# Gustavroot/DeflatedMLMC_Schwinger

Measured on AMD Instinct MI355X. Metric: hutchinson_probe_samples_per_sec_schwinger128, higher is better.
Workload: dtype f64

## Files before the change

### deflatedmlmc_schwinger_amd/csrc/sw_engine.hip

```cpp
#include "../../include/schwinger_hip.h"
#include "sw_kernels.hpp"
#include "sw_pack.hpp"
#include "sw_poly.hpp"

#include <dlfcn.h>

#include <algorithm>
#include <chrono>
#include <cmath>
#include <complex>
#include <cstdarg>
#include <cstdio>
#include <cstdlib>
#include <cstring>
#include <functional>
#include <map>
#include <mutex>
#include <string>
#include <type_traits>
#include <vector>

using swk::cplx;
using swk::cplxf;
using swk::PtrList;
// ... 157 lines not shown
  bool direct_small = true;
  bool lgmres_aug = true;
  bool stencil_nt = false;
  int stencil_tile = 0;
  int stencil_spw = 0;
  bool cgs2 = false;
  bool verify = true;
  bool inner_cgs2 = false;
  bool pyth_last = true;
  bool eo_solve = true;
  bool eo_direct = true;
  bool precond_f32 = false;
  int kd = 0;
  cplx* U = nullptr;
  int defl_gemm = 0;
  int lkd[SW_MAX_LEVELS] = {0};
  cplx* lV[SW_MAX_LEVELS] = {nullptr};
  int* perm_src[SW_MAX_LEVELS] = {nullptr};
  EllOp rhsmap[SW_MAX_LEVELS];
  cplx* partial = nullptr;
  size_t partial_bytes = 0;
  cplx* small = nullptr;
  size_t small_bytes = 0;
  void* stage = nullptr;
  size_t stage_bytes = 0;
  std::vector<std::pair<void*, size_t>> allocs;
  int pb_level = -1, pb_nb = 0, pb_nbp = 0;
  int8_t* pb_probes = nullptr;
  struct ProbeSlot {
    int8_t* p = nullptr;
    size_t bytes = 0;
    int level = -1, nb = 0;
    hipEvent_t ready = nullptr;
    bool pending = false;
  };
  std::vector<ProbeSlot> slots;
  bool mt_set = false;
  uint32_t* mt_win0 = nullptr;
  uint32_t* mt_win = nullptr;
  int mt_cur = 0;
  uint64_t mt_pos = 0;
  uint32_t* mt_poly = nullptr;
  uint64_t mt_dist = 0;
  uint32_t* mt_family = nullptr;
  uint64_t mt_fam_seg = 0;
  int mt_fam_count = 0;
// ... 6 lines not shown
  bool profiling = false;
  std::vector<EventRec> recs;
  std::vector<hipEvent_t> evpool;
  double tacc[T_NCAT] = {0};
  int64_t tcount[T_NCAT] = {0};
  double twork[T_NCAT] = {0};
  int64_t launches = 0;
  int* d_notconv = nullptr;
  int nc_next = 0;
  int* h_notconv = nullptr;
  int* d_tick = nullptr;
  bool fused_reduce = true;
  double stop_factor = 1.0;
  std::vector<double> direct_relres;
  int64_t direct_fallbacks = 0;
  double alloc_s = 0.0, alloc_bytes = 0.0;
  int64_t alloc_calls = 0, pool_hits = 0;
  cplx* eig_buf[3] = {nullptr, nullptr, nullptr};
  signed char* eig_sign = nullptr;
  cplx* eig_small = nullptr;
  int eig_w = 64;
  cplx* eig_cs[2] = {nullptr, nullptr};
  int eig_hid = -1, eig_level = -1, eig_n = 0;
  void* comm = nullptr;
  double* d_stats = nullptr;
};

static int g_dot_blocks = 1024, g_dot_pmax = 1024;

struct EngineOption {
// ... 29 lines not shown
    field<&sw_engine::dense_map>("dense_map", [](double v) { return (int)v >= 0 && (int)v <= 3; },
                                 "dense_map must be 0..3"),
    field<&sw_engine::bsr_sub>("bsr_sub", [](double v) { return (int)v >= 1; }, "bsr_sub must be >= 1"),
    field<&sw_engine::bsr_stages>("bsr_stages", [](double v) { return v == 2.0 || v == 4.0 || v == 8.0; },
                                  "bsr_stages must be 2, 4 or 8 (dense_stages: or 16)"),
    field<&sw_engine::dense_stages>("dense_stages",
                                    [](double v) { return v == 2.0 || v == 4.0 || v == 8.0 || v == 16.0; },
                                    "dense_stages must be 2, 4 or 8 (dense_stages: or 16)"),
    field<&sw_engine::bsr_nt>("bsr_nt"),
    field<&sw_engine::bsr_xreg>("bsr_xreg"),
    {"dense_lds", get_field<&sw_engine::dense_lds>,
     [](sw_engine* h, double v) { h->dense_lds = v == 1.0 ? 2 : (int)v; },
     [](double v) { return v == 0.0 || v == 1.0 || v == 2.0 || v == 4.0; }, "dense_lds must be 0, 2 or 4"},
    field<&sw_engine::defl_gemm>("defl_gemm", [](double v) { return v == 0.0 || v == 1.0; },
                                 "defl_gemm must be 0 or 1"),
    field<&sw_engine::fused_reduce>("fused_reduce"),
    {"dot_blocks", [](const sw_engine*) { return (double)g_dot_blocks; },
     [](sw_engine*, double v) { g_dot_blocks = g_dot_pmax = std::max(64, (int)v); }},
    field<&sw_engine::gj_block>("gj_block",
                                [](double v) {
                                  const int b = (int)v;
                                  return b == 0 || (b >= 8 && b <= 256 && b % 8 == 0);
                                },
                                "gj_block must be 0 or a multiple of 8 in 8..256"),
    field<&sw_engine::stencil_nt>("stencil_nt"),
    field<&sw_engine::stencil_tile>("stencil_tile"),
    field<&sw_engine::stencil_spw>("stencil_spw",
                                   [](double v) {
                                     const int t = (int)v;
                                     return t == 0 || t == 1 || t == 2 || t == 4 || t == 8;
// ... 25 lines not shown
                                   "stop_factor must be in (0, 1]"),
    field<&sw_engine::precond_f32>("precond_f32"),
    field<&sw_engine::f32_krylov>("f32_krylov"),
    field<&sw_engine::f32_pairs>("f32_pairs"),
    field<&sw_engine::f32_tiles>("f32_tiles",
                                 [](double v) { const int t = (int)v; return t == 0 || t == 1 || t == 2 || t == 4; },
                                 "f32_tiles must be 0, 1, 2 or 4"),
    field<&sw_engine::f32_stages>("f32_stages"),
    field<&sw_engine::f32_dense_stages>("f32_dense_stages"),
    field<&sw_engine::f32_splitk>("f32_splitk"),
    field<&sw_engine::bench_what>("bench_what", [](double v) { return !(v < 0.0 || v > 3.0); },
                                  "bench_what must be 0..3"),
    field<&sw_engine::bench_mode>("bench_mode", [](double v) { return v == 0.0 || v == 1.0 || v == 2.0; },
                                  "bench_mode must be 0, 1 or 2"),
    {"direct_fallbacks", get_field<&sw_engine::direct_fallbacks>, nullptr},
    {"alloc_seconds", get_field<&sw_engine::alloc_s>, nullptr},
    {"alloc_calls", get_field<&sw_engine::alloc_calls>, nullptr},
    {"alloc_gbytes", [](const sw_engine* h) { return h->alloc_bytes * 1e-9; }, nullptr},
    {"pool_hits", get_field<&sw_engine::pool_hits>, nullptr},
};

static int sw_fail(sw_engine* h, const char* fmt, ...) {
  char buf[1024];
  va_list ap;
  va_start(ap, fmt);
  vsnprintf(buf, sizeof buf, fmt, ap);
  va_end(ap);
  if (h) h->err = buf;
  else g_create_error = buf;
  return 1;
// ... 864 lines not shown
      const bool even = lv.stencil ? (row < lv.n / 2) : (even_row_tile[row / 16] != 0);
      if (even) ev.push_back(g);
    }
    if (ev.empty()) continue;
    SWCHK(upload(h, &P.order_even, ev.data(), ev.size()));
    P.ngroups_even = (int)ev.size();
  }
  H.even_valid = true;
  return 0;
}

static inline int* sink_slot(sw_engine* h);
static bool f32_capable(const Hier& H, int level);

static int gram_cycle(sw_engine* h, const KrylovSys& sys, const cplx* R, cplx* X, int L, KrylovWS& ws, int nbp,
                      swk::FgTail tg) {
  const size_t vec = (size_t)sys.n * nbp;
  PtrList pu, pz;
  pu.p[0] = R;
  for (int j = 0; j < L; ++j) {
    cplx* z = ws.Z + vec * j;
    cplx* w = ws.V + vec * j;
    SWCHK(sys.precond(pu.p[j], z));
    SWCHK(sys.apply(0, z, nullptr, w));
    pu.p[j + 1] = w;
    pz.p[j] = z;
  }
  tg.kind = SW_TAIL_GRAM;
  tg.s = ws.sc;
  tg.j = L;
  tg.h1 = ws.gram;
  SWCHK(multigram(h, pu, L + 1, sys.n, nbp, ws.gram, &tg));
  return multiaxpy(h, pz, L, ws.sc.ys, 1.0, X, X, sys.n, nbp, nullptr);
}

static int kcycle_gram(sw_engine* h, Hier& H, int level, const cplx* B, cplx* X, int L, KrylovWS& ws, int nbp) {
  swk::FgTail tg{};
  tg.first_cycle = 1;
  tg.notconv = sink_slot(h);
  SWCHK(zero_vec(h, X, H.lv[level].n, nbp));
  return gram_cycle(h, full_system(h, H, level, nbp, true, false), B, X, L, ws, nbp, tg);
}

static int coarse_correction(sw_engine* h, Hier& H, int l, int nbp) {
  Level& lv = H.lv[l];
  Level& lc = H.lv[l + 1];
  const int last = H.nlevels - 1;
  if (lv.kcycle > 0 && l + 1 < last) {
// ... 520 lines not shown
  const int hid_idx = (int)(&H - &h->hier[0]);
  const int check_from = (outer && h->lazy_sync) ? std::max(0, h->sync_hint[hid_idx][level] - 2) : 0;
  const int n = sys.n;
  const size_t vec = (size_t)n * nbp;
  const int tb = 256, tg = (nbp + tb - 1) / tb;
  const double tol_stop = outer ? tol * h->stop_factor : tol;
  const bool z32 = (bool)sys.precond32;
  const bool k32 = z32 && h->f32_krylov;
  if (aug && (outer || sys.precond || ws.m < m + 1)) return sw_fail(h, "internal: augmented cycle misused");
  if (z32 && !(k32 ? (bool)sys.op32 : (bool)sys.op32w))
    return sw_fail(h, "internal: complex64 operator of the Krylov system missing");
  int done = 0;
  bool first = true;
  bool converged = false;
  if (outer) SWCHK(reset_slots(h));
  SWCHK(zero_vec(h, X, n, nbp));
  const cplx* Rcur = B;
  if (z32) {
    Level& lv = H.lv[level];
    SWCHK(ensure_f32(h, H));
    SWCHK(ensure_level_ws32(h, lv, nbp));
    const size_t full = (size_t)lv.n * nbp;
    if (!ws.Z32) {
      SWCHK(dev_realloc(h, &ws.Z32, full * m));
      SWCHK(dev_realloc(h, &ws.v32, full));
    }
    if (k32 && !ws.V32) SWCHK(dev_realloc(h, &ws.V32, full * m));
  }
  while (done < maxiter && !converged) {
    {
      PtrList pl;
// ... 58 lines not shown
      }
      }
      if (outer && tol_stop > 0.0 && (done + j + 1 >= check_from || done + j + 1 >= maxiter ||
                                      ((done + j + 1) & 7) == 0)) {
        int left = 0;
        SWCHK(read_slot(h, slot, &left));
        if (left == 0) {
          converged = true;
          ++j;
          break;
        }
      }
    }
    const int k = j;
    SWCHK(launch(h, T_OTHER, swk::k_fg_solve, dim3(tg), dim3(tb), ws.sc, k));
    if (z32) {
      swk::PtrListT<cplxf> pz;
      for (int q = 0; q < k; ++q) pz.p[q] = ws.Z32 + vec * q;
      SWCHK(multiaxpy(h, pz, k, ws.sc.ys, 1.0, X, X, n, nbp, nullptr));
    } else {
      PtrList pz;
      for (int q = 0; q < k; ++q) pz.p[q] = ws.Z + vec * q;
      SWCHK(multiaxpy(h, pz, k, ws.sc.ys, 1.0, X, X, n, nbp, nullptr));
    }
    done += k;
    first = false;
    if (!outer) break;
    if (converged && h->verify) {
      SWCHK(sys.apply(1, X, B, ws.rres));
      PtrList pr;
      pr.p[0] = ws.rres;
      int* slot = nullptr;
      SWCHK(take_slot(h, &slot));
      const swk::FgTail tv = tail_verify(ws, tol, tol_stop, slot);
      SWCHK(multidot(h, pr, 1, ws.rres, n, nbp, ws.nrm, nullptr, nullptr, &tv));
      int left = 0;
      SWCHK(read_slot(h, slot, &left));
      if (left != 0) {
// ... 202 lines not shown
  if (hid == 0) {
    h->kd = 0;
    SWCHK(dev_free(h, h->U));
    h->U = nullptr;
    for (int l = 0; l < SW_MAX_LEVELS; ++l) {
      h->lkd[l] = 0;
      SWCHK(dev_free(h, h->lV[l]));
      h->lV[l] = nullptr;
      SWCHK(dev_free(h, h->perm_src[l]));
      h->perm_src[l] = nullptr;
      SWCHK(free_op(h, h->rhsmap[l]));
    }
    HIPCHK(hipStreamSynchronize(h->gen_stream));
    for (auto& sl : h->slots) {
      SWCHK(dev_free(h, sl.p));
      if (sl.ready) (void)hipEventDestroy(sl.ready);
    }
    h->slots.clear();
    h->pb_slot = -1;
    h->pb_probes = nullptr;
    h->pb_level = -1;
    h->pb_nb = h->pb_nbp = 0;
    h->pb_ws_nbp = 0;
  }
  return 0;
}

int sw_set_lattice(sw_engine* h, int hid, int L, double mass, const double* U1, const double* U2) {
  SWCHK(check_hier(h, hid, 0, false));
  if (L < 2 || (L & 1)) return sw_fail(h, "lattice extent L=%d must be even and >= 2", L);
// ... 1371 lines not shown
  if (h->precond_f32 && h->f32_krylov && f32_capable(H, 0)) {
    s.precond32 = [h, &H, nbp](const cplxf* v, cplxf* z) { return vcycle32_even(h, H, v, z, nbp); };
    s.op32 = [h, &lv, nbp](const cplxf* z, cplxf* w) { return schur_apply32(h, lv, z, w, nbp); };
  }
  return s;
}

static int reduced_rhs(sw_engine* h, Level& lv, const cplx* B, KrylovWS& ws, int nbp) {
  PtrList pl;
  pl.p[0] = B;
  const swk::FgTail tbeg = tail_begin(ws, 1);
  SWCHK(multidot(h, pl, 1, B, lv.n, nbp, ws.nrm, nullptr, nullptr, &tbeg));
  return eo_hop<0>(h, lv, B, B, ws.xacc, nbp);
}

static int fgmres_eo(sw_engine* h, Hier& H, const cplx* B, cplx* X, double tol, int maxiter, int m,
                     KrylovWS& ws, int nbp, int* iters_total) {
  Level& lv = H.lv[0];
  SWCHK(ensure_level_ws(h, lv, nbp));
  SWCHK(reduced_rhs(h, lv, B, ws, nbp));
  SWCHK(fgmres_loop(h, H, 0, reduced_system(h, H, nbp), ws.xacc, X, tol, maxiter, m, true, ws, nbp,
                    iters_total));
  return eo_hop<1>(h, lv, B, X, X, nbp);
}

static int fgmres_eo_gram(sw_engine* h, Hier& H, const cplx* B, cplx* X, double tol, int maxiter, int m,
                          KrylovWS& ws, int nbp, int* iters_total) {
  Level& lv = H.lv[0];
  const int hid_idx = (int)(&H - &h->hier[0]);
  const int hint = h->lazy_sync ? h->sync_hint[hid_idx][0] : 0;
  const KrylovSys sys = reduced_system(h, H, nbp);
  const double tol_stop = tol * h->stop_factor;
  SWCHK(ensure_level_ws(h, lv, nbp));
  SWCHK(reset_slots(h));
  SWCHK(reduced_rhs(h, lv, B, ws, nbp));
  const cplx* bp = ws.xacc;
  SWCHK(zero_vec(h, X, sys.n, nbp));
  std::vector<std::complex<double>> hrr(nbp), hrr0(nbp);
  int done = 0;
  bool converged = false;
  const cplx* Rcur = bp;
  int L = std::min(m, maxiter);
  while (done < maxiter && !converged) {
    L = std::max(1, std::min(L, std::min(m, maxiter - done)));
    int* slot = nullptr;
    SWCHK(take_slot(h, &slot));
    swk::FgTail tg{};
    tg.tol = tol;
    tg.tol_stop = tol_stop;
    tg.iter_base = done;
    tg.notconv = slot;
    SWCHK(gram_cycle(h, sys, Rcur, X, L, ws, nbp, tg));
    done += L;
    SWCHK(sys.apply(1, X, bp, ws.rres));
    Rcur = ws.rres;
    const bool observe = tol_stop > 0.0 && (hint <= 0 || done + m >= hint || done >= maxiter);
    int Lnext = m;
    if (observe) {
      int left = 0;
      SWCHK(read_slot(h, slot, &left));
      if (left == 0) {
        converged = true;
      } else {
        HIPCHK(hipMemcpy(hrr.data(), ws.sc.relres, sizeof(cplx) * nbp, hipMemcpyDeviceToHost));
        HIPCHK(hipMemcpy(hrr0.data(), ws.sc.g, sizeof(cplx) * nbp, hipMemcpyDeviceToHost));
        double need = 1.0;
        for (int c = 0; c < nbp; ++c) {
// ... 9 lines not shown
      PtrList pr;
      pr.p[0] = ws.rres;
      int* vslot = nullptr;
      SWCHK(take_slot(h, &vslot));
      const swk::FgTail tv = tail_verify(ws, tol, tol_stop, vslot);
      SWCHK(multidot(h, pr, 1, ws.rres, sys.n, nbp, ws.nrm, nullptr, nullptr, &tv));
      int left = 0;
      SWCHK(read_slot(h, vslot, &left));
      if (left != 0) {
        converged = false;
        Lnext = 1;
      }
    }
    L = Lnext;
  }
  SWCHK(eo_hop<1>(h, lv, B, X, X, nbp));
  if (iters_total) *iters_total = done;
  h->sync_hint[hid_idx][0] = converged ? done : 0;
  return 0;
}

static bool level_is_direct(sw_engine* h, Hier& H, int level) {
  return h->direct_small && level < H.nlevels - 1 && !H.lv[level].stencil && H.lv[level].dinv.set &&
         h->use_mfma;
}

static int solve_dev(sw_engine* h, int hid, int level0, const cplx* B, cplx* X, double tol,
                     int maxiter, int nbp, int* total) {
  Hier& H = h->hier[hid];
  Level& lv = H.lv[level0];
  if (level0 == H.nlevels - 1 && H.nlevels > 1) {
    SWCHK(apply_coarsest(h, H, B, X, nbp));
    if (total) *total = 1;
    return 0;
// ... 22 lines not shown
        worst = std::max(worst, rr);
      }
      if (!(worst > tol * h->stop_factor)) return 0;
      if (pass == 3) break;
      SWCHK(launch_bsr(h, lv.dinv, 0, lv.r, nullptr, lv.t, nbp, T_COARSEST, cplx{0.0, 0.0}));
      SWCHK(vec_add(h, X, lv.t, X, lv.n, nbp));
    }
    h->direct_relres.clear();
    h->direct_fallbacks++;
    const int mfb = std::min(h->restart, std::max(1, maxiter));
    SWCHK(ensure_krylov(h, lv.sws, mfb, lv.n, nbp, true));
    return fgmres(h, H, level0, B, X, tol, maxiter, mfb, true, lv.sws, nbp, total);
  }
  const int m = std::min(h->restart, std::max(1, maxiter));
  SWCHK(ensure_krylov(h, lv.sws, m, lv.n, nbp, true));
  if (eo_solve_eligible(h, H, level0)) {
    const bool k32 = h->precond_f32 && h->f32_krylov && f32_capable(H, 0);
    int P = 0, rpb = 0;
    row_blocking(lv.n / 2, nbp, true, &P, &rpb);
    if (h->gram_cycle && !k32 && m <= SW_GRAM_MAXL && fused_ok(h, P, nbp))
      return fgmres_eo_gram(h, H, B, X, tol, maxiter, m, lv.sws, nbp, total);
    return fgmres_eo(h, H, B, X, tol, maxiter, m, lv.sws, nbp, total);
  }
  return fgmres(h, H, level0, B, X, tol, maxiter, m, true, lv.sws, nbp, total);
}

static int fetch_iters(sw_engine* h, KrylovWS& ws, int nb, int32_t* iters, double* relres,
                       int fallback_iters) {
  std::vector<int> it(ws.nbp);
  std::vector<std::complex<double>> rr(ws.nbp);
  HIPCHK(hipMemcpy(it.data(), ws.sc.iters, sizeof(int) * ws.nbp, hipMemcpyDeviceToHost));
  HIPCHK(hipMemcpy(rr.data(), ws.sc.relres, sizeof(cplx) * ws.nbp, hipMemcpyDeviceToHost));
  for (int j = 0; j < nb; ++j) {
    if (iters) iters[j] = it[j] >= 0 ? it[j] : fallback_iters;
    if (relres) relres[j] = rr[j].real();
  }
  return 0;
}
// ... 38 lines not shown
  SWCHK(dev_realloc(h, &h->pb_x0, cnt));
  SWCHK(dev_realloc(h, &h->pb_rhs, cnt));
  SWCHK(dev_realloc(h, &h->pb_z, cnt));
  SWCHK(dev_realloc(h, &h->pb_xc, cnt));
  SWCHK(dev_realloc(h, &h->pb_xc2, cnt));
  SWCHK(dev_realloc(h, &h->pb_y, cnt));
  SWCHK(dev_realloc(h, &h->pb_w, cnt));
  SWCHK(dev_realloc(h, &h->pb_w2, cnt));
  SWCHK(dev_realloc(h, &h->pb_xd, cnt));
  SWCHK(dev_realloc(h, &h->pb_est, (size_t)4 * nbp));
  SWCHK(dev_realloc(h, &h->pb_iters, (size_t)2 * nbp));
  h->pb_ws_nbp = nbp;
  return 0;
}

int sw_probes_upload_slot(sw_engine* h, int slot, int level, int nb, const int8_t* probes) {
  SWCHK(check_hier(h, 0, level, true));
  if (nb <= 0 || !probes) return sw_fail(h, "bad arguments");
  if (slot < 0 || slot >= 4096) return sw_fail(h, "probe slot %d out of range", slot);
  HIPCHK(hipSetDevice(h->device));
  Level& lv = h->hier[0].lv[level];
  const size_t bytes = (size_t)nb * lv.n;
  if ((int)h->slots.size() <= slot) h->slots.resize(slot + 1);
  sw_engine::ProbeSlot& sl = h->slots[slot];
  if (sl.pending) {
    HIPCHK(hipStreamSynchronize(h->gen_stream));
    sl.pending = false;
  }
  if (sl.bytes < bytes) {
    SWCHK(dev_free(h, sl.p));
    sl.p = nullptr;
    void* q;
    SWCHK(dev_alloc(h, &q, bytes));
    sl.p = (int8_t*)q;
    sl.bytes = bytes;
  }
  HIPCHK(hipMemcpyAsync(sl.p, probes, bytes, hipMemcpyHostToDevice, h->stream));
  HIPCHK(hipStreamSynchronize(h->stream));
  sl.level = level;
  sl.nb = nb;
  return 0;
}

int sw_probes_select(sw_engine* h, int slot) {
  if (!h) return 1;
  if (slot < 0 || slot >= (int)h->slots.size() || !h->slots[slot].p)
    return sw_fail(h, "probe slot %d is empty", slot);
  h->pb_slot = slot;
  h->pb_probes = h->slots[slot].p;
  h->pb_level = h->slots[slot].level;
  h->pb_nb = h->slots[slot].nb;
  h->pb_nbp = pad64(h->pb_nb);
  return 0;
}

// ... 86 lines not shown
    void* q;
    SWCHK(dev_alloc(h, &q, total));
    sl.p = (int8_t*)q;
    sl.bytes = total;
  }
  {
    LaunchScope ls(h, T_OTHER);
    hipLaunchKernelGGL(swk::k_mt_generate, dim3(S), dim3(SW_MT_BLOCK), 0, gs,
                       (const uint32_t*)(h->mt_win + (size_t)SW_MT_N * h->mt_cur),
                       (const uint32_t*)h->mt_family, (unsigned long long)segdraws,
                       (unsigned long long)total, kind, sl.p);
    KLAUNCH_CHECK();
  }
  sl.level = level;
  sl.nb = nb;
  if (!sl.ready) HIPCHK(hipEventCreateWithFlags(&sl.ready, hipEventDisableTiming));
  HIPCHK(hipEventRecord(sl.ready, gs));
  sl.pending = true;
  return 0;
}

int sw_probes_fetch(sw_engine* h, int slot, int8_t* out) {
  if (!h) return 1;
  if (!out) return sw_fail(h, "null output");
  if (slot < 0 || slot >= (int)h->slots.size() || !h->slots[slot].p)
    return sw_fail(h, "probe slot %d is empty", slot);
  HIPCHK(hipSetDevice(h->device));
  SWCHK(stream_sync(h));
  HIPCHK(hipStreamSynchronize(h->gen_stream));
  const sw_engine::ProbeSlot& sl = h->slots[slot];
// ... 3 lines not shown
}

static int dot_into(sw_engine* h, const cplx* A, const cplx* Bv, int n, int nbp, cplx* out) {
  PtrList pl;
  pl.p[0] = A;
  return multidot(h, pl, 1, Bv, n, nbp, out);
}

static int record_iters(sw_engine* h, KrylovWS* ws, int total_or_const, std::vector<int32_t>& dst,
                        int nb) {
  dst.assign(nb, total_or_const);
  if (ws) {
    std::vector<int> it(ws->nbp);
    HIPCHK(hipMemcpy(it.data(), ws->sc.iters, sizeof(int) * ws->nbp, hipMemcpyDeviceToHost));
    for (int j = 0; j < nb; ++j) dst[j] = it[j] >= 0 ? it[j] : total_or_const;
  }
  return 0;
}

static int deflate(sw_engine* h, const cplx* U, int kd, const int* srcrow, const cplx* X, cplx* out,
                   int n, int nbp) {
  const int ld = defl_ld(kd);
  cplx* cbuf = h->small + 8 * nbp;
  if (h->defl_gemm || kd > 64) {
    const int nchunks = nbp / 16;
    const int pmax = std::max(1, (n + 63) / 64);
    int P = std::max(1, std::min(pmax, 2048 / nchunks));
    const int rpb = (n + P - 1) / P;
    P = (n + rpb - 1) / rpb;
    SWCHK(ensure_partial(h, (size_t)P * ld * nbp * sizeof(cplx)));
    SWCHK(pick_ge<64, 128, 256>(ld, [&](auto LD) {
      return launch(h, T_DEFL, swk::k_defl_gemm_dots<LD / 64>, dim3(P, nchunks), dim3(SW_BLOCK), U, ld, X, n, nbp,
                    rpb, h->partial);
    }));
    SWCHK(launch(h, T_DEFL, swk::k_reduce_partials, dim3(ld, nbp / 64), dim3(SW_BLOCK), h->partial, P, ld, nbp,
                 cbuf, (const cplx*)nullptr, (cplx*)nullptr));
    return launch(h, T_DEFL, swk::k_defl_gemm_apply, dim3((n + 63) / 64, nbp / 64), dim3(SW_BLOCK), U, ld,
                  (const cplx*)cbuf, srcrow, X, out, n, nbp);
  }
  int P, rpb;
  row_blocking(n, nbp, true, &P, &rpb);
  for (int k0 = 0; k0 < kd; k0 += 32) {
    const int kc = std::min(32, kd - k0);
    SWCHK(ensure_partial(h, (size_t)P * kc * nbp * sizeof(cplx)));
    SWCHK(pick_ge<8, 16, 32>(kc, [&](auto KC) {
      return launch(h, T_DEFL, swk::k_defl_dots<KC>, dim3(P, nbp / 64), dim3(SW_BLOCK), (const cplx*)(U + k0), ld,
                    kc, X, n, nbp, rpb, h->partial);
    }));
    SWCHK(launch(h, T_DEFL, swk::k_reduce_partials, dim3(kc, nbp / 64), dim3(SW_BLOCK), h->partial, P, kc, nbp,
                 cbuf + (size_t)k0 * nbp, (const cplx*)nullptr, (cplx*)nullptr));
  }
  {
    dim3 grid((n + SW_WAVES_PER_BLOCK - 1) / SW_WAVES_PER_BLOCK, nbp / 64);
    SWCHK(launch(h, T_DEFL, swk::k_defl_apply, grid, dim3(SW_BLOCK), U, ld, kd, cbuf, srcrow, X, out, n, nbp));
  }
  return 0;
}

int sw_apply_deflation(sw_engine* h, int which, int level, int nb, const double* X, double* Y) {
  SWCHK(check_hier(h, 0, level, false));
  if (which != 0 && which != 1) return sw_fail(h, "which must be 0 (Hutchinson) or 1 (MLMC level)");
  if (which == 0 && level != 0) return sw_fail(h, "the Hutchinson deflation acts at level 0");
  if (nb <= 0 || !X || !Y) return sw_fail(h, "bad arguments");
  const int kd = which == 0 ? h->kd : h->lkd[level];
  const cplx* U = which == 0 ? h->U : h->lV[level];
  if (kd <= 0 || !U) return sw_fail(h, "no deflation vectors registered at level %d", level);
  HIPCHK(hipSetDevice(h->device));
  Level& lv = h->hier[0].lv[level];
  const int nbp = pad64(nb);
  cplx *a, *b;
  SWCHK(io_vectors(h, lv, nbp, &a, &b));
  SWCHK(ensure_small(h, nbp));
  SWCHK(pack_host(h, lv, nb, X, a, nbp));
  SWCHK(deflate(h, U, kd, which == 0 ? (const int*)h->perm_src[0] : nullptr, a, b, lv.n, nbp));
  return unpack_host(h, lv, nb, b, Y, nbp);
}

int sw_hutch_run(sw_engine* h, int mode, int level, double tol, int maxiter) {
  SWCHK(check_hier(h, 0, level, true));
  if (h->pb_level != level || h->pb_nb <= 0) return sw_fail(h, "no probes uploaded for level %d", level);
  if (maxiter < 1) return sw_fail(h, "maxiter must be >= 1");
  HIPCHK(hipSetDevice(h->device));
  Hier& H0 = h->hier[0];
  const int nb = h->pb_nb, nbp = h->pb_nbp;
  Level& lv = H0.lv[level];
  const int n = lv.n;
  SWCHK(ensure_probe_ws(h, nbp));
  SWCHK(ensure_small(h, nbp));
  if (h->pb_slot >= 0 && h->pb_slot < (int)h->slots.size() && h->slots[h->pb_slot].pending) {
    HIPCHK(hipStreamWaitEvent(h->stream, h->slots[h->pb_slot].ready, 0));
    h->slots[h->pb_slot].pending = false;
  }
  SWCHK(launch(h, T_OTHER, swk::k_pack_i8, dim3((n + 63) / 64, nbp / 64), dim3(SW_BLOCK), h->pb_probes, nb, n,
               (const int*)lv.rowmap, h->pb_x0, nbp));
  const int fine_hid = (level == 0 && h->hier[h->solver_hid].ready) ? h->solver_hid : 0;
  if (fine_hid != 0 && h->hier[fine_hid].lv[0].n != n)
    return sw_fail(h, "solver hierarchy level-0 size mismatch");
  if (mode == SW_MODE_HUTCHINSON) {
    if (level != 0) return sw_fail(h, "Hutchinson mode runs at level 0");
    const int kd = h->kd;
    if (kd > 0) {
      SWCHK(deflate(h, h->U, kd, (const int*)h->perm_src[0], h->pb_x0, h->pb_rhs, n, nbp));
    } else {
      dim3 grid((n + SW_WAVES_PER_BLOCK - 1) / SW_WAVES_PER_BLOCK, nbp / 64);
      SWCHK(launch(h, T_DEFL, swk::k_gather_rows, grid, dim3(SW_BLOCK), (const int*)h->perm_src[0], h->pb_x0,
                   h->pb_rhs, n, nbp));
    }
    int total = 0;
    SWCHK(solve_dev(h, fine_hid, 0, h->pb_rhs, h->pb_z, tol, maxiter, nbp, &total));
    SWCHK(dot_into(h, h->pb_x0, h->pb_z, n, nbp, h->pb_est));
    SWCHK(stream_sync(h));
    SWCHK(record_iters(h, &h->hier[fine_hid].lv[0].sws, total, h->last_iters_f, nb));
// ... 283 lines not shown
```

### deflatedmlmc_schwinger_amd/csrc/sw_kernels.hpp

```cpp
#pragma once
#include <hip/hip_runtime.h>
#include <stdint.h>

namespace swk {

typedef double2 cplx;

#define SW_WAVE 64
#define SW_BLOCK 256
#define SW_WAVES_PER_BLOCK 4

__device__ __forceinline__ cplx cmake(double a, double b) { cplx r; r.x = a; r.y = b; return r; }
__device__ __forceinline__ cplx cadd(cplx a, cplx b) { return cmake(a.x + b.x, a.y + b.y); }
__device__ __forceinline__ cplx csub(cplx a, cplx b) { return cmake(a.x - b.x, a.y - b.y); }
__device__ __forceinline__ cplx cmul(cplx a, cplx b) {
  return cmake(fma(a.x, b.x, -a.y * b.y), fma(a.x, b.y, a.y * b.x));
}
__device__ __forceinline__ cplx cmulc(cplx a, cplx b) {
  return cmake(fma(a.x, b.x, a.y * b.y), fma(a.x, b.y, -a.y * b.x));
}
__device__ __forceinline__ void cfma(cplx& acc, cplx a, cplx b) {
  acc.x = fma(a.x, b.x, acc.x);
  acc.x = fma(-a.y, b.y, acc.x);
  acc.y = fma(a.x, b.y, acc.y);
// ... 2131 lines not shown
  const int r1 = min(n, r0 + rows_per_block);
  cplx c[KT];
#pragma unroll
  for (int k = 0; k < KT; ++k) {
    c[k] = cmake(0.0, 0.0);
    if (k < K) {
      const cplx t = coef[(size_t)k * nbp + col];
      c[k] = cmake(sign * t.x, sign * t.y);
    }
  }
  double nrm = 0.0;
  constexpr int UNR = (sizeof(CV) == sizeof(cplxf) && sizeof(CW) == sizeof(cplxf)) ? 4 : 2;
#pragma unroll UNR
  for (int r = r0 + wave; r < r1; r += SW_WAVES_PER_BLOCK) {
    const size_t off = (size_t)r * nbp + col;
    cplx w = widen(Win[off]);
#pragma unroll
    for (int k = 0; k < KT; ++k)
      if (k < K) cfma(w, c[k], widen(V.p[k][off]));
    Wout[off] = narrow<CW>(w);
    if (W32) W32[off] = cmake((float)w.x, (float)w.y);
    if (NORM) nrm = fma(w.x, w.x, fma(w.y, w.y, nrm));
  }
  if (NORM) {
    if (wave > 0) redn[wave - 1][lane] = nrm;
    __syncthreads();
    if (wave == 0) {
      nrm += redn[0][lane];
      nrm += redn[1][lane];
      nrm += redn[2][lane];
      st_partial(&partial[(size_t)blockIdx.x * nbp + col], cmake(nrm, 0.0), ra.tick1 != nullptr);
// ... 36 lines not shown
  const size_t stride = (size_t)gridDim.x * blockDim.x;
  for (; i < count; i += stride) dst[i] = cadd(a[i], b[i]);
}

__global__ __launch_bounds__(SW_BLOCK) void k_gather_rows(const int* __restrict__ srcrow,
                                                          const cplx* __restrict__ src,
                                                          cplx* __restrict__ dst, int n, int nbp) {
  const int wave = threadIdx.x >> 6, lane = threadIdx.x & 63;
  const size_t col = (size_t)blockIdx.y * 64 + lane;
  const int r = blockIdx.x * SW_WAVES_PER_BLOCK + wave;
  if (r >= n) return;
  const int s = srcrow ? srcrow[r] : r;
  dst[(size_t)r * nbp + col] = src[(size_t)s * nbp + col];
}

template <int KT>
__global__ __launch_bounds__(SW_BLOCK) void k_defl_dots(const cplx* __restrict__ U, int ldu,
                                                        int kd, const cplx* __restrict__ X, int n,
                                                        int nbp, int rows_per_block,
                                                        cplx* __restrict__ partial) {
  __shared__ cplx red[3][8][64];
  const int wave = threadIdx.x >> 6, lane = threadIdx.x & 63;
  const size_t col = (size_t)blockIdx.y * 64 + lane;
  const int r0 = blockIdx.x * rows_per_block;
  const int r1 = min(n, r0 + rows_per_block);
  cplx acc[KT];
#pragma unroll
  for (int k = 0; k < KT; ++k) acc[k] = cmake(0.0, 0.0);
  for (int r = r0 + wave; r < r1; r += SW_WAVES_PER_BLOCK) {
    const int ru = __builtin_amdgcn_readfirstlane(r);
    const cplx x = X[(size_t)ru * nbp + col];
    const cplx* u = U + (size_t)ru * ldu;
#pragma unroll
    for (int k = 0; k < KT; ++k)
      if (k < kd) cfmac(acc[k], u[k], x);
  }
  for (int kb = 0; kb < KT; kb += 8) {
    if (kb >= kd) break;
    if (wave > 0) {
#pragma unroll
      for (int k = 0; k < 8; ++k)
        if (kb + k < KT) red[wave - 1][k][lane] = acc[kb + k];
    }
    __syncthreads();
    if (wave == 0) {
#pragma unroll
// ... 17 lines not shown
                                                         const cplx* __restrict__ X,
                                                         cplx* __restrict__ out, int n, int nbp) {
  const int wave = threadIdx.x >> 6, lane = threadIdx.x & 63;
  const size_t col = (size_t)blockIdx.y * 64 + lane;
  const int r = __builtin_amdgcn_readfirstlane(blockIdx.x * SW_WAVES_PER_BLOCK + wave);
  if (r >= n) return;
  const int s = srcrow ? srcrow[r] : r;
  cplx x = X[(size_t)s * nbp + col];
  const cplx* u = U + (size_t)s * ldu;
#pragma unroll 4
  for (int k = 0; k < kd; ++k) {
    const cplx ck = c[(size_t)k * nbp + col];
    cfma(x, cmake(-u[k].x, -u[k].y), ck);
  }
  out[(size_t)r * nbp + col] = x;
}

template <int KT>
__global__ __launch_bounds__(SW_BLOCK) void k_defl_gemm_dots(const cplx* __restrict__ U, int ldu,
                                                             const cplx* __restrict__ X, int n, int nbp,
                                                             int rows_per_block,
                                                             cplx* __restrict__ partial) {
  const int lane = threadIdx.x & 63, wave = threadIdx.x >> 6;
  const int k = lane >> 4, c = lane & 15;
  const int t0 = wave * KT;
  const int nt = min(KT, ldu / 16 - t0);
  if (nt <= 0) return;
  const int r0 = blockIdx.x * rows_per_block;
  const int r1 = min(n, r0 + rows_per_block);
  const size_t j = (size_t)blockIdx.y * 16 + c;
// ... 436 lines not shown
```

Measured before the change: 35450.

## Add fused Hutchinson probe path with int8 probe image and fused deflation/EO kernels

Adds a dedicated Hutchinson path for level 0. Probe vectors stay in a pre-transposed, row-mapped int8 image built when probes are uploaded, possibly on the generator stream. Deflation dots read the int8 probes directly. A fused kernel builds the deflated, even-odd reduced right-hand side together with its norm, and another fused kernel reconstructs the odd sites and accumulates the trace estimate. This replaces the separate pack, deflate-apply, reduced-rhs, hop and dot launches and their full complex-vector traffic. The first FGMRES cycle also skips zeroing X and reading it back in the axpy. The cost is more kernel code, an extra per-slot buffer, and an eligibility check that falls back to the old path.

```diff
diff --git a/deflatedmlmc_schwinger_amd/csrc/sw_engine.hip b/deflatedmlmc_schwinger_amd/csrc/sw_engine.hip
--- a/deflatedmlmc_schwinger_amd/csrc/sw_engine.hip
+++ b/deflatedmlmc_schwinger_amd/csrc/sw_engine.hip
@@ -195,6 +195,7 @@
   int kd = 0;
   cplx* U = nullptr;
   int defl_gemm = 0;
+  bool probe_path = true;
   int lkd[SW_MAX_LEVELS] = {0};
   cplx* lV[SW_MAX_LEVELS] = {nullptr};
   int* perm_src[SW_MAX_LEVELS] = {nullptr};
@@ -211,6 +212,9 @@
   struct ProbeSlot {
     int8_t* p = nullptr;
     size_t bytes = 0;
+    int8_t* xt = nullptr;
+    size_t xt_bytes = 0;
+    bool xt_ok = false;
     int level = -1, nb = 0;
     hipEvent_t ready = nullptr;
     bool pending = false;
@@ -247,6 +251,7 @@
   double stop_factor = 1.0;
   std::vector<double> direct_relres;
   int64_t direct_fallbacks = 0;
+  int64_t probe_batches = 0;
   double alloc_s = 0.0, alloc_bytes = 0.0;
   int64_t alloc_calls = 0, pool_hits = 0;
   cplx* eig_buf[3] = {nullptr, nullptr, nullptr};
@@ -306,6 +311,7 @@
      [](double v) { return v == 0.0 || v == 1.0 || v == 2.0 || v == 4.0; }, "dense_lds must be 0, 2 or 4"},
     field<&sw_engine::defl_gemm>("defl_gemm", [](double v) { return v == 0.0 || v == 1.0; },
                                  "defl_gemm must be 0 or 1"),
+    field<&sw_engine::probe_path>("probe_path"),
     field<&sw_engine::fused_reduce>("fused_reduce"),
     {"dot_blocks", [](const sw_engine*) { return (double)g_dot_blocks; },
      [](sw_engine*, double v) { g_dot_blocks = g_dot_pmax = std::max(64, (int)v); }},
@@ -361,6 +367,7 @@
     field<&sw_engine::bench_mode>("bench_mode", [](double v) { return v == 0.0 || v == 1.0 || v == 2.0; },
                                   "bench_mode must be 0, 1 or 2"),
     {"direct_fallbacks", get_field<&sw_engine::direct_fallbacks>, nullptr},
+    {"probe_batches", get_field<&sw_engine::probe_batches>, nullptr},
     {"alloc_seconds", get_field<&sw_engine::alloc_s>, nullptr},
     {"alloc_calls", get_field<&sw_engine::alloc_calls>, nullptr},
     {"alloc_gbytes", [](const sw_engine* h) { return h->alloc_bytes * 1e-9; }, nullptr},
@@ -1255,7 +1262,7 @@
 static bool f32_capable(const Hier& H, int level);
 
 static int gram_cycle(sw_engine* h, const KrylovSys& sys, const cplx* R, cplx* X, int L, KrylovWS& ws, int nbp,
-                      swk::FgTail tg) {
+                      swk::FgTail tg, bool first = false) {
   const size_t vec = (size_t)sys.n * nbp;
   PtrList pu, pz;
   pu.p[0] = R;
@@ -1272,7 +1279,7 @@
   tg.j = L;
   tg.h1 = ws.gram;
   SWCHK(multigram(h, pu, L + 1, sys.n, nbp, ws.gram, &tg));
-  return multiaxpy(h, pz, L, ws.sc.ys, 1.0, X, X, sys.n, nbp, nullptr);
+  return multiaxpy(h, pz, L, ws.sc.ys, 1.0, first ? (const cplx*)nullptr : X, X, sys.n, nbp, nullptr);
 }
 
 static int kcycle_gram(sw_engine* h, Hier& H, int level, const cplx* B, cplx* X, int L, KrylovWS& ws, int nbp) {
@@ -1823,7 +1830,7 @@
   bool first = true;
   bool converged = false;
   if (outer) SWCHK(reset_slots(h));
-  SWCHK(zero_vec(h, X, n, nbp));
+  if (!outer) SWCHK(zero_vec(h, X, n, nbp));
   const cplx* Rcur = B;
   if (z32) {
     Level& lv = H.lv[level];
@@ -1912,14 +1919,15 @@
     }
     const int k = j;
     SWCHK(launch(h, T_OTHER, swk::k_fg_solve, dim3(tg), dim3(tb), ws.sc, k));
+    const cplx* x0 = (outer && first) ? nullptr : X;
     if (z32) {
       swk::PtrListT<cplxf> pz;
       for (int q = 0; q < k; ++q) pz.p[q] = ws.Z32 + vec * q;
-      SWCHK(multiaxpy(h, pz, k, ws.sc.ys, 1.0, X, X, n, nbp, nullptr));
+      SWCHK(multiaxpy(h, pz, k, ws.sc.ys, 1.0, x0, X, n, nbp, nullptr));
     } else {
       PtrList pz;
       for (int q = 0; q < k; ++q) pz.p[q] = ws.Z + vec * q;
-      SWCHK(multiaxpy(h, pz, k, ws.sc.ys, 1.0, X, X, n, nbp, nullptr));
+      SWCHK(multiaxpy(h, pz, k, ws.sc.ys, 1.0, x0, X, n, nbp, nullptr));
     }
     done += k;
     first = false;
@@ -2152,6 +2160,7 @@
     HIPCHK(hipStreamSynchronize(h->gen_stream));
     for (auto& sl : h->slots) {
       SWCHK(dev_free(h, sl.p));
+      SWCHK(dev_free(h, sl.xt));
       if (sl.ready) (void)hipEventDestroy(sl.ready);
     }
     h->slots.clear();
@@ -3553,28 +3562,20 @@
   return eo_hop<0>(h, lv, B, B, ws.xacc, nbp);
 }
 
-static int fgmres_eo(sw_engine* h, Hier& H, const cplx* B, cplx* X, double tol, int maxiter, int m,
-                     KrylovWS& ws, int nbp, int* iters_total) {
-  Level& lv = H.lv[0];
-  SWCHK(ensure_level_ws(h, lv, nbp));
-  SWCHK(reduced_rhs(h, lv, B, ws, nbp));
-  SWCHK(fgmres_loop(h, H, 0, reduced_system(h, H, nbp), ws.xacc, X, tol, maxiter, m, true, ws, nbp,
-                    iters_total));
-  return eo_hop<1>(h, lv, B, X, X, nbp);
-}
-
-static int fgmres_eo_gram(sw_engine* h, Hier& H, const cplx* B, cplx* X, double tol, int maxiter, int m,
-                          KrylovWS& ws, int nbp, int* iters_total) {
-  Level& lv = H.lv[0];
+static int fgmres_eo_loop(sw_engine* h, Hier& H, cplx* X, double tol, int maxiter, int m, KrylovWS& ws, int nbp,
+                          int* iters_total) {
+  return fgmres_loop(h, H, 0, reduced_system(h, H, nbp), ws.xacc, X, tol, maxiter, m, true, ws, nbp,
+                     iters_total);
+}
+
+static int fgmres_eo_gram_loop(sw_engine* h, Hier& H, cplx* X, double tol, int maxiter, int m, KrylovWS& ws,
+                               int nbp, int* iters_total) {
   const int hid_idx = (int)(&H - &h->hier[0]);
   const int hint = h->lazy_sync ? h->sync_hint[hid_idx][0] : 0;
   const KrylovSys sys = reduced_system(h, H, nbp);
   const double tol_stop = tol * h->stop_factor;
-  SWCHK(ensure_level_ws(h, lv, nbp));
   SWCHK(reset_slots(h));
-  SWCHK(reduced_rhs(h, lv, B, ws, nbp));
   const cplx* bp = ws.xacc;
-  SWCHK(zero_vec(h, X, sys.n, nbp));
   std::vector<std::complex<double>> hrr(nbp), hrr0(nbp);
   int done = 0;
   bool converged = false;
@@ -3589,7 +3590,7 @@
     tg.tol_stop = tol_stop;
     tg.iter_base = done;
     tg.notconv = slot;
-    SWCHK(gram_cycle(h, sys, Rcur, X, L, ws, nbp, tg));
+    SWCHK(gram_cycle(h, sys, Rcur, X, L, ws, nbp, tg, done == 0));
     done += L;
     SWCHK(sys.apply(1, X, bp, ws.rres));
     Rcur = ws.rres;
@@ -3629,10 +3630,28 @@
     }
     L = Lnext;
   }
-  SWCHK(eo_hop<1>(h, lv, B, X, X, nbp));
   if (iters_total) *iters_total = done;
   h->sync_hint[hid_idx][0] = converged ? done : 0;
   return 0;
+}
+
+static int eo_loop(sw_engine* h, Hier& H, cplx* X, double tol, int maxiter, int m, KrylovWS& ws, int nbp,
+                   int* iters_total) {
+  const bool k32 = h->precond_f32 && h->f32_krylov && f32_capable(H, 0);
+  int P = 0, rpb = 0;
+  row_blocking(H.lv[0].n / 2, nbp, true, &P, &rpb);
+  if (h->gram_cycle && !k32 && m <= SW_GRAM_MAXL && fused_ok(h, P, nbp))
+    return fgmres_eo_gram_loop(h, H, X, tol, maxiter, m, ws, nbp, iters_total);
+  return fgmres_eo_loop(h, H, X, tol, maxiter, m, ws, nbp, iters_total);
+}
+
+static int solve_eo(sw_engine* h, Hier& H, const cplx* B, cplx* X, double tol, int maxiter, int m, KrylovWS& ws,
+                    int nbp, int* iters_total) {
+  Level& lv = H.lv[0];
+  SWCHK(ensure_level_ws(h, lv, nbp));
+  SWCHK(reduced_rhs(h, lv, B, ws, nbp));
+  SWCHK(eo_loop(h, H, X, tol, maxiter, m, ws, nbp, iters_total));
+  return eo_hop<1>(h, lv, B, X, X, nbp);
 }
 
 static bool level_is_direct(sw_engine* h, Hier& H, int level) {
@@ -3685,14 +3704,7 @@
   }
   const int m = std::min(h->restart, std::max(1, maxiter));
   SWCHK(ensure_krylov(h, lv.sws, m, lv.n, nbp, true));
-  if (eo_solve_eligible(h, H, level0)) {
-    const bool k32 = h->precond_f32 && h->f32_krylov && f32_capable(H, 0);
-    int P = 0, rpb = 0;
-    row_blocking(lv.n / 2, nbp, true, &P, &rpb);
-    if (h->gram_cycle && !k32 && m <= SW_GRAM_MAXL && fused_ok(h, P, nbp))
-      return fgmres_eo_gram(h, H, B, X, tol, maxiter, m, lv.sws, nbp, total);
-    return fgmres_eo(h, H, B, X, tol, maxiter, m, lv.sws, nbp, total);
-  }
+  if (eo_solve_eligible(h, H, level0)) return solve_eo(h, H, B, X, tol, maxiter, m, lv.sws, nbp, total);
   return fgmres(h, H, level0, B, X, tol, maxiter, m, true, lv.sws, nbp, total);
 }
 
@@ -3761,6 +3773,29 @@
   return 0;
 }
 
+static int probe_image(sw_engine* h, sw_engine::ProbeSlot& sl, hipStream_t st) {
+  Level& lv = h->hier[0].lv[sl.level];
+  const int nbp = pad64(sl.nb);
+  const size_t need = (size_t)lv.n * nbp;
+  if (sl.xt_bytes < need) {
+    HIPCHK(hipStreamSynchronize(h->stream));
+    HIPCHK(hipStreamSynchronize(h->gen_stream));
+    SWCHK(dev_free(h, sl.xt));
+    sl.xt = nullptr;
+    sl.xt_bytes = 0;
+    void* q;
+    SWCHK(dev_alloc(h, &q, need));
+    sl.xt = (int8_t*)q;
+    sl.xt_bytes = need;
+  }
+  LaunchScope ls(h, T_OTHER);
+  hipLaunchKernelGGL(swk::k_probe_image, dim3((lv.n + 63) / 64, nbp / 64), dim3(SW_BLOCK), 0, st,
+                     (const int8_t*)sl.p, sl.nb, lv.n, (const int*)lv.rowmap, sl.xt, nbp);
+  KLAUNCH_CHECK();
+  sl.xt_ok = true;
+  return 0;
+}
+
 int sw_probes_upload_slot(sw_engine* h, int slot, int level, int nb, const int8_t* probes) {
   SWCHK(check_hier(h, 0, level, true));
   if (nb <= 0 || !probes) return sw_fail(h, "bad arguments");
@@ -3786,6 +3821,8 @@
   HIPCHK(hipStreamSynchronize(h->stream));
   sl.level = level;
   sl.nb = nb;
+  sl.xt_ok = false;
+  if (h->probe_path && level == 0) SWCHK(probe_image(h, sl, h->stream));
   return 0;
 }
 
@@ -3902,6 +3939,8 @@
   }
   sl.level = level;
   sl.nb = nb;
+  sl.xt_ok = false;
+  if (h->probe_path && level == 0) SWCHK(probe_image(h, sl, gs));
   if (!sl.ready) HIPCHK(hipEventCreateWithFlags(&sl.ready, hipEventDisableTiming));
   HIPCHK(hipEventRecord(sl.ready, gs));
   sl.pending = true;
@@ -3935,6 +3974,24 @@
     std::vector<int> it(ws->nbp);
     HIPCHK(hipMemcpy(it.data(), ws->sc.iters, sizeof(int) * ws->nbp, hipMemcpyDeviceToHost));
     for (int j = 0; j < nb; ++j) dst[j] = it[j] >= 0 ? it[j] : total_or_const;
+  }
+  return 0;
+}
+
+extern "C++" template <class XT>
+static int defl_dots(sw_engine* h, const cplx* U, int kd, const XT* X, int n, int nbp, cplx* cbuf) {
+  const int ld = defl_ld(kd);
+  int P, rpb;
+  row_blocking(n, nbp, true, &P, &rpb);
+  for (int k0 = 0; k0 < kd; k0 += 32) {
+    const int kc = std::min(32, kd - k0);
+    SWCHK(ensure_partial(h, (size_t)P * kc * nbp * sizeof(cplx)));
+    SWCHK(pick_ge<8, 16, 32>(kc, [&](auto KC) {
+      return launch(h, T_DEFL, swk::k_defl_dots<KC, XT>, dim3(P, nbp / 64), dim3(SW_BLOCK), (const cplx*)(U + k0), ld,
+                    kc, X, n, nbp, rpb, h->partial);
+    }));
+    SWCHK(launch(h, T_DEFL, swk::k_reduce_partials, dim3(kc, nbp / 64), dim3(SW_BLOCK), h->partial, P, kc, nbp,
+                 cbuf + (size_t)k0 * nbp, (const cplx*)nullptr, (cplx*)nullptr));
   }
   return 0;
 }
@@ -3959,18 +4016,7 @@
     return launch(h, T_DEFL, swk::k_defl_gemm_apply, dim3((n + 63) / 64, nbp / 64), dim3(SW_BLOCK), U, ld,
                   (const cplx*)cbuf, srcrow, X, out, n, nbp);
   }
-  int P, rpb;
-  row_blocking(n, nbp, true, &P, &rpb);
-  for (int k0 = 0; k0 < kd; k0 += 32) {
-    const int kc = std::min(32, kd - k0);
-    SWCHK(ensure_partial(h, (size_t)P * kc * nbp * sizeof(cplx)));
-    SWCHK(pick_ge<8, 16, 32>(kc, [&](auto KC) {
-      return launch(h, T_DEFL, swk::k_defl_dots<KC>, dim3(P, nbp / 64), dim3(SW_BLOCK), (const cplx*)(U + k0), ld,
-                    kc, X, n, nbp, rpb, h->partial);
-    }));
-    SWCHK(launch(h, T_DEFL, swk::k_reduce_partials, dim3(kc, nbp / 64), dim3(SW_BLOCK), h->partial, P, kc, nbp,
-                 cbuf + (size_t)k0 * nbp, (const cplx*)nullptr, (cplx*)nullptr));
-  }
+  SWCHK(defl_dots(h, U, kd, X, n, nbp, cbuf));
   {
     dim3 grid((n + SW_WAVES_PER_BLOCK - 1) / SW_WAVES_PER_BLOCK, nbp / 64);
     SWCHK(launch(h, T_DEFL, swk::k_defl_apply, grid, dim3(SW_BLOCK), U, ld, kd, cbuf, srcrow, X, out, n, nbp));
@@ -3997,6 +4043,63 @@
   return unpack_host(h, lv, nb, b, Y, nbp);
 }
 
+static int probe_site_blocking(int Vh, int* P) {
+  int spb = std::max(SW_WAVES_PER_BLOCK, (Vh + 255) / 256);
+  spb = (spb + SW_WAVES_PER_BLOCK - 1) / SW_WAVES_PER_BLOCK * SW_WAVES_PER_BLOCK;
+  *P = (Vh + spb - 1) / spb;
+  return spb;
+}
+
+static bool probe_path_eligible(sw_engine* h, Hier& H, int nbp) {
+  if (!h->probe_path || h->kd > 32 || (h->kd > 0 && h->defl_gemm) || h->pb_slot < 0 ||
+      h->pb_slot >= (int)h->slots.size() || h->slots[h->pb_slot].level != 0)
+    return false;
+  if (!eo_solve_eligible(h, H, 0) || (h->precond_f32 && h->f32_krylov && f32_capable(H, 0))) return false;
+  int P = 0;
+  probe_site_blocking(H.lv[0].L * H.lv[0].L / 2, &P);
+  return fused_ok(h, P, nbp);
+}
+
+static int hutch_probe_path(sw_engine* h, Hier& H, double tol, int maxiter) {
+  sw_engine::ProbeSlot& sl = h->slots[h->pb_slot];
+  const int nb = h->pb_nb, nbp = h->pb_nbp, kd = h->kd;
+  Level& lv = H.lv[0];
+  const int n = lv.n;
+  if (!sl.xt_ok) SWCHK(probe_image(h, sl, h->stream));
+  h->probe_batches++;
+  const int m = std::min(h->restart, std::max(1, maxiter));
+  SWCHK(ensure_krylov(h, lv.sws, m, n, nbp, true));
+  SWCHK(ensure_level_ws(h, lv, nbp));
+  KrylovWS& ws = lv.sws;
+  cplx* cbuf = h->small + 8 * nbp;
+  if (kd > 0) SWCHK(defl_dots(h, h->U, kd, (const int8_t*)sl.xt, n, nbp, cbuf));
+  const swk::StencilArgs a = stencil_args<cplx>(h, lv, nbp, true);
+  int P = 0;
+  const int spb = probe_site_blocking(a.Vh, &P);
+  const int ngroups = (P + SW_RED_GROUP - 1) / SW_RED_GROUP;
+  const dim3 grid(P, nbp / 64);
+  const double di = 1.0 / a.diag;
+  const int* srcrow = (const int*)h->perm_src[0];
+  SWCHK(ensure_partial(h, (size_t)(P + ngroups) * nbp * sizeof(cplx)));
+  {
+    const swk::RedArgs ra = red_args(h, true, P, 1, nbp, ws.nrm, nullptr, nullptr);
+    SWCHK(launch(h, T_DEFL, swk::k_probe_rhs, grid, dim3(SW_BLOCK), (const int8_t*)sl.xt, (const cplx*)h->U,
+                 defl_ld(kd), kd, (const cplx*)cbuf, srcrow, ws.xacc, a, di, spb, h->partial, ra, tail_begin(ws, 1)));
+  }
+  int total = 0;
+  SWCHK(eo_loop(h, H, h->pb_z, tol, maxiter, m, ws, nbp, &total));
+  {
+    const swk::RedArgs ra = red_args(h, true, P, 1, nbp, h->pb_est, nullptr, nullptr);
+    SWCHK(launch(h, T_OTHER, swk::k_probe_est, grid, dim3(SW_BLOCK), (const int8_t*)sl.xt, (const cplx*)h->U,
+                 defl_ld(kd), kd, (const cplx*)cbuf, srcrow, (const cplx*)h->pb_z, a, di, spb, h->partial, ra,
+                 kNoTail));
+  }
+  SWCHK(stream_sync(h));
+  SWCHK(record_iters(h, &ws, total, h->last_iters_f, nb));
+  h->last_iters_c.assign(nb, 0);
+  return 0;
+}
+
 int sw_hutch_run(sw_engine* h, int mode, int level, double tol, int maxiter) {
   SWCHK(check_hier(h, 0, level, true));
   if (h->pb_level != level || h->pb_nb <= 0) return sw_fail(h, "no probes uploaded for level %d", level);
@@ -4012,11 +4115,13 @@
     HIPCHK(hipStreamWaitEvent(h->stream, h->slots[h->pb_slot].ready, 0));
     h->slots[h->pb_slot].pending = false;
   }
-  SWCHK(launch(h, T_OTHER, swk::k_pack_i8, dim3((n + 63) / 64, nbp / 64), dim3(SW_BLOCK), h->pb_probes, nb, n,
-               (const int*)lv.rowmap, h->pb_x0, nbp));
   const int fine_hid = (level == 0 && h->hier[h->solver_hid].ready) ? h->solver_hid : 0;
   if (fine_hid != 0 && h->hier[fine_hid].lv[0].n != n)
     return sw_fail(h, "solver hierarchy level-0 size mismatch");
+  if (mode == SW_MODE_HUTCHINSON && level == 0 && probe_path_eligible(h, h->hier[fine_hid], nbp))
+    return hutch_probe_path(h, h->hier[fine_hid], tol, maxiter);
+  SWCHK(launch(h, T_OTHER, swk::k_pack_i8, dim3((n + 63) / 64, nbp / 64), dim3(SW_BLOCK), h->pb_probes, nb, n,
+               (const int*)lv.rowmap, h->pb_x0, nbp));
   if (mode == SW_MODE_HUTCHINSON) {
     if (level != 0) return sw_fail(h, "Hutchinson mode runs at level 0");
     const int kd = h->kd;
diff --git a/deflatedmlmc_schwinger_amd/csrc/sw_kernels.hpp b/deflatedmlmc_schwinger_amd/csrc/sw_kernels.hpp
--- a/deflatedmlmc_schwinger_amd/csrc/sw_kernels.hpp
+++ b/deflatedmlmc_schwinger_amd/csrc/sw_kernels.hpp
@@ -2169,7 +2169,7 @@
 #pragma unroll UNR
   for (int r = r0 + wave; r < r1; r += SW_WAVES_PER_BLOCK) {
     const size_t off = (size_t)r * nbp + col;
-    cplx w = widen(Win[off]);
+    cplx w = Win ? widen(Win[off]) : cmake(0.0, 0.0);
 #pragma unroll
     for (int k = 0; k < KT; ++k)
       if (k < K) cfma(w, c[k], widen(V.p[k][off]));
@@ -2236,9 +2236,15 @@
   dst[(size_t)r * nbp + col] = src[(size_t)s * nbp + col];
 }
 
-template <int KT>
+__device__ __forceinline__ cplx probe_decode(int v) {
+  return (v == 2 || v == -2) ? cmake(0.0, (double)(v / 2)) : cmake((double)v, 0.0);
+}
+__device__ __forceinline__ cplx ld_probe(const cplx* p) { return *p; }
+__device__ __forceinline__ cplx ld_probe(const int8_t* p) { return probe_decode(*p); }
+
+template <int KT, class XT = cplx>
 __global__ __launch_bounds__(SW_BLOCK) void k_defl_dots(const cplx* __restrict__ U, int ldu,
-                                                        int kd, const cplx* __restrict__ X, int n,
+                                                        int kd, const XT* __restrict__ X, int n,
                                                         int nbp, int rows_per_block,
                                                         cplx* __restrict__ partial) {
   __shared__ cplx red[3][8][64];
@@ -2251,7 +2257,7 @@
   for (int k = 0; k < KT; ++k) acc[k] = cmake(0.0, 0.0);
   for (int r = r0 + wave; r < r1; r += SW_WAVES_PER_BLOCK) {
     const int ru = __builtin_amdgcn_readfirstlane(r);
-    const cplx x = X[(size_t)ru * nbp + col];
+    const cplx x = ld_probe(&X[(size_t)ru * nbp + col]);
     const cplx* u = U + (size_t)ru * ldu;
 #pragma unroll
     for (int k = 0; k < KT; ++k)
@@ -2299,6 +2305,155 @@
     cfma(x, cmake(-u[k].x, -u[k].y), ck);
   }
   out[(size_t)r * nbp + col] = x;
+}
+
+__global__ __launch_bounds__(SW_BLOCK) void k_probe_image(const int8_t* __restrict__ src, int nb, int n,
+                                                          const int* __restrict__ rowmap,
+                                                          int8_t* __restrict__ dst, int nbp) {
+  __shared__ int8_t tile[64][65];
+  const int i0 = blockIdx.x * 64;
+  const int j0 = blockIdx.y * 64;
+  const int tx = threadIdx.x & 63, ty = threadIdx.x >> 6;
+  for (int jj = ty; jj < 64; jj += 4) {
+    const int j = j0 + jj, i = i0 + tx;
+    tile[jj][tx] = (j < nb && i < n) ? src[(size_t)j * n + i] : (int8_t)0;
+  }
+  __syncthreads();
+  for (int ii = ty; ii < 64; ii += 4) {
+    const int i = i0 + ii;
+    if (i < n) {
+      const size_t row = rowmap ? (size_t)rowmap[i] : (size_t)i;
+      dst[row * nbp + j0 + tx] = tile[tx][ii];
+    }
+  }
+}
+
+template <int NS>
+__device__ __forceinline__ void probe_rhs_sites(const int8_t* __restrict__ xt, const cplx* __restrict__ U,
+                                                int ldu, int kd, const cplx* __restrict__ c,
+                                                const int* __restrict__ srcrow, const size_t (&row)[NS],
+                                                int nbp, size_t col, Site2 (&b)[NS]) {
+  const cplx* u[2 * NS];
+  cplx x[2 * NS];
+#pragma unroll
+  for (int i = 0; i < 2 * NS; ++i) {
+    const size_t r = row[i >> 1] + (i & 1);
+    const size_t s = srcrow ? (size_t)srcrow[r] : r;
+    x[i] = probe_decode(xt[s * nbp + col]);
+    u[i] = U + s * ldu;
+  }
+#pragma unroll 2
+  for (int k = 0; k < kd; ++k) {
+    const cplx ck = c[(size_t)k * nbp + col];
+#pragma unroll
+    for (int i = 0; i < 2 * NS; ++i) cfma(x[i], cmake(-u[i][k].x, -u[i][k].y), ck);
+  }
+#pragma unroll
+  for (int i = 0; i < NS; ++i) {
+    b[i].s0 = x[2 * i];
+    b[i].s1 = x[2 * i + 1];
+  }
+}
+
+__global__ __launch_bounds__(SW_BLOCK) void k_probe_rhs(const int8_t* __restrict__ xt,
+                                                        const cplx* __restrict__ U, int ldu, int kd,
+                                                        const cplx* __restrict__ c,
+                                                        const int* __restrict__ srcrow, cplx* __restrict__ out,
+                                                        StencilArgs a, double beta, int spb,
+                                                        cplx* __restrict__ partial, RedArgs ra, FgTail tail) {
+  __shared__ double redn[3][64];
+  __shared__ cplx redt[256];
+  const int wave = threadIdx.x >> 6, lane = threadIdx.x & 63;
+  const int L = a.L, Vh = a.Vh, nbp = a.nbp;
+  const size_t col = (size_t)blockIdx.y * 64 + lane;
+  const int s0 = blockIdx.x * spb, s1 = min(Vh, s0 + spb);
+  double nrm = 0.0;
+  for (int sh = s0 + wave; sh < s1; sh += SW_WAVES_PER_BLOCK) {
+    const int su = __builtin_amdgcn_readfirstlane(sh);
+    int x, y;
+    eo_site(su, 0, L, a.tile_w, 0, L, x, y);
+    const int xp = wrap_p(x, L), xm = wrap_m(x, L), yp = wrap_p(y, L), ym = wrap_m(y, L);
+    const size_t r = eo_row(x, y, L, Vh);
+    const size_t row[5] = {r, eo_row(xp, y, L, Vh), eo_row(xm, y, L, Vh), eo_row(x, yp, L, Vh),
+                           eo_row(x, ym, L, Vh)};
+    Site2 b[5];
+    probe_rhs_sites<5>(xt, U, ldu, kd, c, srcrow, row, nbp, col, b);
+    Site2 acc;
+    acc.s0 = czero<cplx>();
+    acc.s1 = acc.s0;
+    hop_acc<0>(acc, a.U1[y * L + x], b[1]);
+    hop_acc<1>(acc, a.U1[y * L + xm], b[2]);
+    hop_acc<2>(acc, a.U2[y * L + x], b[3]);
+    hop_acc<3>(acc, a.U2[ym * L + x], b[4]);
+    out[r * nbp + col] = clin(1.0, b[0].s0, beta, acc.s0);
+    out[(r + 1) * nbp + col] = clin(1.0, b[0].s1, beta, acc.s1);
+#pragma unroll
+    for (int i = 0; i < 2; ++i) {
+      nrm = fma(b[i].s0.x, b[i].s0.x, fma(b[i].s0.y, b[i].s0.y, nrm));
+      nrm = fma(b[i].s1.x, b[i].s1.x, fma(b[i].s1.y, b[i].s1.y, nrm));
+    }
+  }
+  if (wave > 0) redn[wave - 1][lane] = nrm;
+  __syncthreads();
+  if (wave == 0) {
+    nrm += redn[0][lane];
+    nrm += redn[1][lane];
+    nrm += redn[2][lane];
+    st_partial(&partial[(size_t)blockIdx.x * nbp + col], cmake(nrm, 0.0), ra.tick1 != nullptr);
+  }
+  if (ra.tick1) reduce_and_tail<1>(partial, 1, nbp, ra, tail, redt);
+}
+
+__global__ __launch_bounds__(SW_BLOCK) void k_probe_est(const int8_t* __restrict__ xt,
+                                                        const cplx* __restrict__ U, int ldu, int kd,
+                                                        const cplx* __restrict__ c,
+                                                        const int* __restrict__ srcrow,
+                                                        const cplx* __restrict__ X, StencilArgs a, double di,
+                                                        int spb, cplx* __restrict__ partial, RedArgs ra,
+                                                        FgTail tail) {
+  __shared__ cplx rede[3][64];
+  __shared__ cplx redt[256];
+  const int wave = threadIdx.x >> 6, lane = threadIdx.x & 63;
+  const int L = a.L, Vh = a.Vh, nbp = a.nbp;
+  const size_t col = (size_t)blockIdx.y * 64 + lane;
+  const int s0 = blockIdx.x * spb, s1 = min(Vh, s0 + spb);
+  const cplx* S = X + col;
+  const int8_t* x0 = xt + col;
+  cplx e = cmake(0.0, 0.0);
+  for (int sh = s0 + wave; sh < s1; sh += SW_WAVES_PER_BLOCK) {
+    const int su = __builtin_amdgcn_readfirstlane(sh);
+    int x, y;
+    eo_site(su, 1, L, a.tile_w, 0, L, x, y);
+    const int xp = wrap_p(x, L), xm = wrap_m(x, L), yp = wrap_p(y, L), ym = wrap_m(y, L);
+    const size_t r = eo_row(x, y, L, Vh);
+    const size_t row[1] = {r};
+    Site2 b[1];
+    probe_rhs_sites<1>(xt, U, ldu, kd, c, srcrow, row, nbp, col, b);
+    const Site2 ex = ld_site(S, xp, y, L, Vh, nbp);
+    Site2 acc;
+    acc.s0 = czero<cplx>();
+    acc.s1 = acc.s0;
+    hop_acc<0>(acc, a.U1[y * L + x], ex);
+    hop_acc<1>(acc, a.U1[y * L + xm], ld_site(S, xm, y, L, Vh, nbp));
+    hop_acc<2>(acc, a.U2[y * L + x], ld_site(S, x, yp, L, Vh, nbp));
+    hop_acc<3>(acc, a.U2[ym * L + x], ld_site(S, x, ym, L, Vh, nbp));
+    const cplx xo0 = clin(di, b[0].s0, di, acc.s0);
+    const cplx xo1 = clin(di, b[0].s1, di, acc.s1);
+    const size_t re = eo_row(xp, y, L, Vh);
+    cfmac(e, probe_decode(x0[r * nbp]), xo0);
+    cfmac(e, probe_decode(x0[(r + 1) * nbp]), xo1);
+    cfmac(e, probe_decode(x0[re * nbp]), ex.s0);
+    cfmac(e, probe_decode(x0[(re + 1) * nbp]), ex.s1);
+  }
+  if (wave > 0) rede[wave - 1][lane] = e;
+  __syncthreads();
+  if (wave == 0) {
+    e = cadd(e, rede[0][lane]);
+    e = cadd(e, rede[1][lane]);
+    e = cadd(e, rede[2][lane]);
+    st_partial(&partial[(size_t)blockIdx.x * nbp + col], e, ra.tick1 != nullptr);
+  }
+  if (ra.tick1) reduce_and_tail<1>(partial, 1, nbp, ra, tail, redt);
 }
 
 template <int KT>
```

New measurement: 35890, median of 6. +1.3%, better.
